# Cameronr11/GAN-Variant-Research

Measured on AMD Instinct MI355X. Metric: images/sec (G+D train step) 256x256 CUT, higher is better.
Workload: dtype bf16; 1 GPU; CUT ResNet-9 G + PatchGAN D + PatchNCE + identity + lazy R1 + DiffAugment, 256x256, batch 16 per GPU (BASELINE.json configs[2]); global_batch=16, parallelism=dp1

## Files before the change

### gan-variant-research_amd/csrc/conv_win7.hip

```cpp
#include "common.h"

namespace {

constexpr int TS = 16, PW = TS + 6, PITCH = 144, PATCH_BYTES = PW * PW * PITCH;
constexpr int NJ = 4;

struct Win7Args {
  const char* in; const char* w; const float* bias; char* out;
  int B, Ho, Wo, tiles_x, tiles_y;
  int in_Hp, in_Wp, in_y0, in_x0, ty0, tx0;
  int out_Hp, out_Wp, out_y0, out_x0;
  int act;
  float* stats;
};

__global__ __launch_bounds__(256, 2) void conv_win7_kernel(Win7Args a) {
  extern __shared__ __attribute__((aligned(16))) char lds[];
  const int tid = threadIdx.x, lane = tid & 63, wave = __builtin_amdgcn_readfirstlane(tid >> 6);
  const int G = gridDim.x;
  const int q = G >> 3, r = G & 7, xcd = blockIdx.x & 7, k = blockIdx.x >> 3;
  const int tile = xcd < r ? xcd * (q + 1) + k : r * (q + 1) + (xcd - r) * q + k;
  const int per_img = a.tiles_x * a.tiles_y;
  const int b = tile / per_img, t2 = tile - b * per_img;
  const int oy0 = (t2 / a.tiles_x) * TS, ox0 = (t2 % a.tiles_x) * TS;

  u32x4_t bw[NJ][7];
  {
    const char* wl = a.w + (lane & 15) * (49 * 128) + (lane >> 4) * 16;
#pragma unroll
    for (int j = 0; j < NJ; ++j) {
      const int id = wave + 4 * j, kx = min(id >> 1, 6), c = id & 1;
#pragma unroll
      for (int ky = 0; ky < 7; ++ky) {
        u32x4_t v = *reinterpret_cast<const u32x4_t*>(wl + (ky * 7 + kx) * 128 + c * 64);
        if (id >= 14) v = u32x4_t{0u, 0u, 0u, 0u};
        bw[j][ky] = v;
      }
    }
  }
  {
    const int ay0 = oy0 + a.in_y0 + a.ty0, ax0 = ox0 + a.in_x0 + a.tx0;
    const char* img = a.in + (int64_t)b * a.in_Hp * a.in_Wp * 128;
    constexpr int NIT = (PW * PW * 8 + 255) / 256;
    u32x4_t st[NIT];
#pragma unroll
    for (int it = 0; it < NIT; ++it) {
      const int i = tid + it * 256;
      const int p = i >> 3, ck = i & 7;
      const int py = p / PW, px = p - py * PW;
      const int ay = ay0 + py, ax = ax0 + px;
      const bool ok = i < PW * PW * 8 && ay >= 0 && ay < a.in_Hp && ax >= 0 && ax < a.in_Wp;
      const int64_t off = ok ? ((int64_t)ay * a.in_Wp + ax) * 128 + ck * 16 : 0;
      u32x4_t v = *reinterpret_cast<const u32x4_t*>(img + off);
      if (!ok) v = u32x4_t{0u, 0u, 0u, 0u};
      st[it] = v;
    }
#pragma unroll
    for (int it = 0; it < NIT; ++it) {
      const int i = tid + it * 256;
      if (i < PW * PW * 8) *reinterpret_cast<u32x4_t*>(lds + (i >> 3) * PITCH + (i & 7) * 16) = st[it];
    }
  }
  __syncthreads();

  f32x4_t acc[TS];
#pragma unroll
  for (int m = 0; m < TS; ++m) acc[m] = f32x4_t{0.f, 0.f, 0.f, 0.f};
  const char* la = lds + (lane & 15) * PITCH + (lane >> 4) * 16;
#pragma unroll
  for (int j = 0; j < NJ; ++j) {
    const int id = wave + 4 * j, kx = min(id >> 1, 6), c = id & 1;
    const char* lj = la + kx * PITCH + c * 64;
#pragma unroll
    for (int R = 0; R < PW; ++R) {
      const u32x4_t xa = *reinterpret_cast<const u32x4_t*>(lj + R * (PW * PITCH));
#pragma unroll
      for (int ky = 0; ky < 7; ++ky) {
        const int m = R - ky;
        if (m >= 0 && m < TS)
          acc[m] = __builtin_amdgcn_mfma_f32_16x16x32_bf16(__builtin_bit_cast(bf16x8_t, bw[j][ky]), __builtin_bit_cast(bf16x8_t, xa), acc[m], 0, 0, 0);
      }
    }
    __builtin_amdgcn_sched_barrier(0);
  }
  __syncthreads();
  {
    float* red = reinterpret_cast<float*>(lds);
#pragma unroll
    for (int m = 0; m < TS; ++m)
      *reinterpret_cast<f32x4_t*>(red + (((wave * TS + m) * TS + (lane & 15)) * 16 + (lane >> 4) * 4)) = acc[m];
  }
  __syncthreads();
  {
    const float* red = reinterpret_cast<const float*>(lds);
    const int m = tid >> 4, x = tid & 15;
    float v[8];
#pragma unroll
    for (int n = 0; n < 8; ++n) v[n] = a.bias ? a.bias[n] : 0.f;
#pragma unroll
    for (int w2 = 0; w2 < 4; ++w2) {
      const f32x4_t p0 = *reinterpret_cast<const f32x4_t*>(red + (((w2 * TS + m) * TS + x) * 16));
      const f32x4_t p1 = *reinterpret_cast<const f32x4_t*>(red + (((w2 * TS + m) * TS + x) * 16 + 4));
      v[0] += p0.x; v[1] += p0.y; v[2] += p0.z; v[3] += p0.w; v[4] += p1.x; v[5] += p1.y; v[6] += p1.z; v[7] += p1.w;
    }
    const int oy = oy0 + m, ox = ox0 + x;
    if (oy < a.Ho && ox < a.Wo) {
#pragma unroll
      for (int n = 0; n < 8; ++n) v[n] = act_apply(v[n], a.act);
      bf16_t* o = reinterpret_cast<bf16_t*>(a.out) + (((int64_t)b * a.out_Hp + oy + a.out_y0) * a.out_Wp + ox + a.out_x0) * 8;
      Chunk<bf16_t>::store(o, v);
    }
  }
}
__device__ __forceinline__ float row16_sum_w7(float v) {
  auto dpp = [](float x, auto ctrl) {
    return __builtin_bit_cast(float, __builtin_amdgcn_update_dpp(0, __builtin_bit_cast(int, x), decltype(ctrl)::value, 0xf, 0xf, true));
  };
  v += dpp(v, std::integral_constant<int, 0xB1>{});
  v += dpp(v, std::integral_constant<int, 0x4E>{});
  v += dpp(v, std::integral_constant<int, 0x141>{});
  v += dpp(v, std::integral_constant<int, 0x140>{});
  return v;
}

constexpr int KS3 = 13;

__global__ __launch_bounds__(256, 2) void conv_win7_from3_kernel(Win7Args a, int wtaps) {
  __shared__ __attribute__((aligned(16))) char lds[(PW * PW + 16) * 16];
  const int tid = threadIdx.x, lane = tid & 63, wave = __builtin_amdgcn_readfirstlane(tid >> 6);
  const int G = gridDim.x;
  const int q = G >> 3, r = G & 7, xcd = blockIdx.x & 7, k = blockIdx.x >> 3;
  const int tile = xcd < r ? xcd * (q + 1) + k : r * (q + 1) + (xcd - r) * q + k;
  const int per_img = a.tiles_x * a.tiles_y;
  const int b = tile / per_img, t2 = tile - b * per_img;
  const int oy0 = (t2 / a.tiles_x) * TS, ox0 = (t2 % a.tiles_x) * TS;
  u32x4_t bw[KS3];
  {
    const char* wl = a.w + ((int64_t)(wave * 16 + (lane & 15)) * wtaps + (lane >> 4)) * 16;
#pragma unroll
    for (int ks = 0; ks < KS3; ++ks) bw[ks] = *reinterpret_cast<const u32x4_t*>(wl + ks * 64);
  }
  {
    const int ay0 = oy0 + a.in_y0 + a.ty0, ax0 = ox0 + a.in_x0 + a.tx0;
    const char* img = a.in + (int64_t)b * a.in_Hp * a.in_Wp * 16;
    u32x4_t st[2];
#pragma unroll
    for (int it = 0; it < 2; ++it) {
      const int p = tid + it * 256;
      const int py = p / PW, px = p - py * PW;
      const int ay = ay0 + py, ax = ax0 + px;
      const bool ok = p < PW * PW && ay >= 0 && ay < a.in_Hp && ax >= 0 && ax < a.in_Wp;
      u32x4_t v = *reinterpret_cast<const u32x4_t*>(img + (ok ? ((int64_t)ay * a.in_Wp + ax) * 16 : 0));
      if (!ok) v = u32x4_t{0u, 0u, 0u, 0u};
      st[it] = v;
    }
#pragma unroll
    for (int it = 0; it < 2; ++it)
      if (tid + it * 256 < PW * PW + 16) *reinterpret_cast<u32x4_t*>(lds + (tid + it * 256) * 16) = st[it];
  }
  __syncthreads();
  f32x4_t acc[TS];
#pragma unroll
  for (int m = 0; m < TS; ++m) acc[m] = f32x4_t{0.f, 0.f, 0.f, 0.f};
  const int g = lane >> 4;
#pragma unroll
  for (int ks = 0; ks < KS3; ++ks) {
    const int t = min(4 * ks + g, 48);
    const int ky = t / 7, kx = t - ky * 7;
    const char* lj = lds + ((ky * PW + kx) + (lane & 15)) * 16;
#pragma unroll
    for (int m = 0; m < TS; ++m) {
      const u32x4_t xa = *reinterpret_cast<const u32x4_t*>(lj + m * (PW * 16));
      acc[m] = __builtin_amdgcn_mfma_f32_16x16x32_bf16(__builtin_bit_cast(bf16x8_t, bw[ks]), __builtin_bit_cast(bf16x8_t, xa), acc[m], 0, 0, 0);
    }
    __builtin_amdgcn_sched_barrier(0);
  }
  const int n0 = wave * 16 + g * 4, x = lane & 15;
  float bias[4];
#pragma unroll
  for (int i = 0; i < 4; ++i) bias[i] = a.bias ? a.bias[n0 + i] : 0.f;
  bf16_t* dst = reinterpret_cast<bf16_t*>(a.out) + (((int64_t)b * a.out_Hp + oy0 + a.out_y0) * a.out_Wp + ox0 + x + a.out_x0) * 64 + n0;
  const bool xok = ox0 + x < a.Wo;
  float ssum[4] = {0.f, 0.f, 0.f, 0.f}, ssq[4] = {0.f, 0.f, 0.f, 0.f};
#pragma unroll
  for (int m = 0; m < TS; ++m) {
    const float v0 = acc[m].x + bias[0], v1 = acc[m].y + bias[1], v2 = acc[m].z + bias[2], v3 = acc[m].w + bias[3];
    uint2 o;
    o.x = (uint32_t)f2bf(v0) | ((uint32_t)f2bf(v1) << 16);
    o.y = (uint32_t)f2bf(v2) | ((uint32_t)f2bf(v3) << 16);
    if (xok && oy0 + m < a.Ho) {
      *reinterpret_cast<uint2*>(dst + (int64_t)m * a.out_Wp * 64) = o;
      ssum[0] += v0; ssum[1] += v1; ssum[2] += v2; ssum[3] += v3;
      ssq[0] += v0 * v0; ssq[1] += v1 * v1; ssq[2] += v2 * v2; ssq[3] += v3 * v3;
    }
  }
  if (a.stats) {
#pragma unroll
    for (int i = 0; i < 4; ++i) { ssum[i] = row16_sum_w7(ssum[i]); ssq[i] = row16_sum_w7(ssq[i]); }
    if (x == 0) {
      float* sp = a.stats + (((int64_t)b * per_img + t2) * 64 + n0) * 2;
#pragma unroll
      for (int i = 0; i < 4; ++i) *reinterpret_cast<float2*>(sp + 2 * i) = make_float2(ssum[i], ssq[i]);
    }
  }
}
}

extern "C" int gan_conv_win7_ok(const gan_conv_desc* d) {
  if (!d || d->dtype != GAN_BF16) return 0;
  const bool to3 = d->Cin == 64 && d->ntaps == 49 && d->Nw == 16 && d->Nst == 8 && d->out_C == 8;
  const bool from3 = d->Cin == 8 && d->ntaps >= 52 && d->Nw == 64 && d->Nst == 64 && d->out_C == 64;
  if (!to3 && !from3) return 0;
  if (d->in_sy != 1 || d->in_sx != 1 || d->out_sy != 1 || d->out_sx != 1 || d->mask || (d->stats && !from3)) return 0;
  if (d->act != GAN_ACT_NONE && !(to3 && d->act == GAN_ACT_TANH)) return 0;
  if (d->max_tapoff != ((d->win_ty0 + 6) * d->in_Wp + d->win_tx0 + 6) * d->Cin) return 0;
  { const char* e = getenv("GAN_NO_WIN7"); if (e && atoi(e)) return 0; }
  return 1;
}

int gan_conv_win7_stats_parts(const gan_conv_desc* d) {
  if (d->w_layout != 2 || d->Cin != 8 || d->Nst != 64 || d->act != GAN_ACT_NONE) return 0;
  return ((d->Wo + TS - 1) / TS) * ((d->Ho + TS - 1) / TS);
}

int gan_conv_win7_launch(const gan_conv_desc* d, hipStream_t s) {
  GAN_CHECK(gan_conv_win7_ok(d), "conv: w_layout 2 set on a descriptor the 7x7 window kernel does not cover");
  GAN_CHECK(d->in_y0 + d->win_ty0 >= 0 && d->in_x0 + d->win_tx0 >= 0 && d->Ho - 1 + d->in_y0 + d->win_ty0 + 6 < d->in_Hp &&
                d->Wo - 1 + d->in_x0 + d->win_tx0 + 6 < d->in_Wp, "conv(7x7 window): taps reach outside the input allocation");
  Win7Args a;
  a.in = (const char*)d->in; a.w = (const char*)d->w; a.bias = d->bias; a.out = (char*)d->out;
  a.B = d->B; a.Ho = d->Ho; a.Wo = d->Wo; a.tiles_x = (d->Wo + TS - 1) / TS; a.tiles_y = (d->Ho + TS - 1) / TS;
  a.in_Hp = d->in_Hp; a.in_Wp = d->in_Wp; a.in_y0 = d->in_y0; a.in_x0 = d->in_x0; a.ty0 = d->win_ty0; a.tx0 = d->win_tx0;
  a.out_Hp = d->out_Hp; a.out_Wp = d->out_Wp; a.out_y0 = d->out_y0; a.out_x0 = d->out_x0;
  a.act = d->act; a.stats = d->stats;
  const int64_t blocks = (int64_t)d->B * a.tiles_x * a.tiles_y;
  GAN_CHECK(blocks < (1ll << 31), "conv(7x7 window): too many tiles");
  static bool attr_set = false;
  if (!attr_set) {
    if (hipFuncSetAttribute((const void*)conv_win7_kernel, hipFuncAttributeMaxDynamicSharedMemorySize, PATCH_BYTES + 64) != hipSuccess)
      return gan_set_error(-2, "conv(7x7 window): cannot raise the dynamic LDS limit to %d bytes", PATCH_BYTES + 64);
    attr_set = true;
  }
  if (d->Cin == 8) {
    hipLaunchKernelGGL(conv_win7_from3_kernel, dim3((unsigned)blocks), dim3(256), 0, s, a, d->ntaps);
    GAN_LAUNCH_CHECK();
    return 0;
  }
  hipLaunchKernelGGL(conv_win7_kernel, dim3((unsigned)blocks), dim3(256), PATCH_BYTES + 64, s, a);
  GAN_LAUNCH_CHECK();
  return 0;
}

namespace {

struct Wg7Args {
  const char* x; const char* g; float* part;
  int B, Ho, Wo, tiles_x, tiles_y, ntiles;
  int x_Hp, x_Wp, x_y0, x_x0;
  int g_Hp, g_Wp, g_y0, g_x0;
};

constexpr int GP = 32;
constexpr int WPITCH = 160, WPATCH = PW * PW * WPITCH;
constexpr int WG7_LDS = WPATCH + 64 + TS * TS * GP;

typedef __attribute__((ext_vector_type(4))) short s16x4_t;

__global__ __launch_bounds__(256, 1) void wgrad_win7_kernel(Wg7Args a) {
  extern __shared__ __attribute__((aligned(16))) char lds[];
  char* lx = lds;
  char* lg = lds + WPATCH + 64;
  const int tid = threadIdx.x, lane = tid & 63, wave = __builtin_amdgcn_readfirstlane(tid >> 6);
  const int fi = lane & 15, fg = lane >> 4, q = fi >> 2, p = fi & 3;
  f32x4_t acc[49];
#pragma unroll
  for (int t = 0; t < 49; ++t) acc[t] = f32x4_t{0.f, 0.f, 0.f, 0.f};
  const int per_img = a.tiles_x * a.tiles_y;
  int xoff[2], goff[2];
#pragma unroll
  for (int h = 0; h < 2; ++h) {
    const int r = fg >> 1, xx = h * 8 + (fg & 1) * 4 + q;
    xoff[h] = (r * PW + xx) * WPITCH + (wave * 16 + p * 4) * 2;
    goff[h] = (r * TS + xx) * GP + p * 8;
  }
  constexpr int NIT = (PW * PW * 8 + 255) / 256;
  u32x4_t st[NIT], gv;
  auto fetch = [&](int tile) {
    const int b = tile / per_img, t2 = tile - b * per_img;
    const int oy0 = (t2 / a.tiles_x) * TS, ox0 = (t2 % a.tiles_x) * TS;
    const int ay0 = oy0 + a.x_y0, ax0 = ox0 + a.x_x0;
    const char* img = a.x + (int64_t)b * a.x_Hp * a.x_Wp * 128;
#pragma unroll
    for (int it = 0; it < NIT; ++it) {
      const int i = tid + it * 256;
      const int px_ = i >> 3, ck = i & 7;
      const int py = px_ / PW, px = px_ - py * PW;
      const int ay = ay0 + py, ax = ax0 + px;
      const bool ok = i < PW * PW * 8 && ay >= 0 && ay < a.x_Hp && ax >= 0 && ax < a.x_Wp;
      u32x4_t v = *reinterpret_cast<const u32x4_t*>(img + (ok ? ((int64_t)ay * a.x_Wp + ax) * 128 + ck * 16 : 0));
      if (!ok) v = u32x4_t{0u, 0u, 0u, 0u};
      st[it] = v;
    }
    const int gy = oy0 + (tid >> 4), gx = ox0 + (tid & 15);
    gv = u32x4_t{0u, 0u, 0u, 0u};
    if (gy < a.Ho && gx < a.Wo) gv = *reinterpret_cast<const u32x4_t*>(a.g + (((int64_t)b * a.g_Hp + gy + a.g_y0) * a.g_Wp + gx + a.g_x0) * 16);
  };
  if ((int)blockIdx.x < a.ntiles) fetch(blockIdx.x);
  for (int tile = blockIdx.x; tile < a.ntiles; tile += gridDim.x) {
    __syncthreads();
#pragma unroll
    for (int it = 0; it < NIT; ++it) {
      const int i = tid + it * 256;
      if (i < PW * PW * 8) *reinterpret_cast<u32x4_t*>(lx + (i >> 3) * WPITCH + (i & 7) * 16) = st[it];
    }
    *reinterpret_cast<u32x4_t*>(lg + tid * GP) = gv;
    *reinterpret_cast<u32x4_t*>(lg + tid * GP + 16) = u32x4_t{0u, 0u, 0u, 0u};
    __syncthreads();
    if (tile + (int)gridDim.x < a.ntiles) fetch(tile + gridDim.x);
    bf16x8_t gfr[8];
#pragma unroll
    for (int ks = 0; ks < 8; ++ks) {
      const s16x4_t g0 = __builtin_amdgcn_ds_read_tr16_b64_v4i16((__attribute__((address_space(3))) s16x4_t*)(lg + ks * (2 * TS * GP) + goff[0]));
      const s16x4_t g1 = __builtin_amdgcn_ds_read_tr16_b64_v4i16((__attribute__((address_space(3))) s16x4_t*)(lg + ks * (2 * TS * GP) + goff[1]));
      gfr[ks] = bf16x8_t{g0[0], g0[1], g0[2], g0[3], g1[0], g1[1], g1[2], g1[3]};
    }
#pragma unroll
    for (int R = 0; R <= 20; ++R) {
#pragma unroll
      for (int kx = 0; kx < 7; ++kx) {
        const int tb = (R * PW + kx) * WPITCH;
        const s16x4_t x0 = __builtin_amdgcn_ds_read_tr16_b64_v4i16((__attribute__((address_space(3))) s16x4_t*)(lx + tb + xoff[0]));
        const s16x4_t x1 = __builtin_amdgcn_ds_read_tr16_b64_v4i16((__attribute__((address_space(3))) s16x4_t*)(lx + tb + xoff[1]));
        const bf16x8_t xv = {x0[0], x0[1], x0[2], x0[3], x1[0], x1[1], x1[2], x1[3]};
#pragma unroll
        for (int ky = R & 1; ky < 7; ky += 2) {
          const int ks = (R - ky) / 2;
          if (R - ky >= 0 && ks < 8) acc[ky * 7 + kx] = __builtin_amdgcn_mfma_f32_16x16x32_bf16(xv, gfr[ks], acc[ky * 7 + kx], 0, 0, 0);
        }
      }
      __builtin_amdgcn_sched_barrier(0);
    }
  }
  if (fi < 8) {
    float* dst = a.part + ((int64_t)blockIdx.x * 8 + fi) * (49 * 64) + wave * 16 + fg * 4;
#pragma unroll
    for (int t = 0; t < 49; ++t) *reinterpret_cast<f32x4_t*>(dst + t * 64) = acc[t];
  }
}
}

namespace {
constexpr int GP64 = 160;
constexpr int XW_BYTES = (PW * PW + 8) * 16;
constexpr int WG7B_LDS = XW_BYTES + TS * TS * GP64;

__global__ __launch_bounds__(256, 2) void wgrad_win7_from3_kernel(Wg7Args a) {
  __shared__ __attribute__((aligned(16))) char lds[WG7B_LDS];
  char* lx = lds;
  char* lg = lds + XW_BYTES;
  const int tid = threadIdx.x, lane = tid & 63, wave = __builtin_amdgcn_readfirstlane(tid >> 6);
  const int fi = lane & 15, fg = lane >> 4, q = fi >> 2, p = fi & 3;
  f32x4_t acc[7][4];
#pragma unroll
  for (int ky = 0; ky < 7; ++ky)
#pragma unroll
    for (int pr = 0; pr < 4; ++pr) acc[ky][pr] = f32x4_t{0.f, 0.f, 0.f, 0.f};
  const int per_img = a.tiles_x * a.tiles_y;
  int xoff[2], goff[2];
#pragma unroll
  for (int h = 0; h < 2; ++h) {
    const int r = fg >> 1, xx = h * 8 + (fg & 1) * 4 + q;
    xoff[h] = (r * PW + xx) * 16 + p * 8;
    goff[h] = (r * TS + xx) * GP64 + (wave * 16 + p * 4) * 2;
  }
  for (int tile = blockIdx.x; tile < a.ntiles; tile += gridDim.x) {
    const int b = tile / per_img, t2 = tile - b * per_img;
    const int oy0 = (t2 / a.tiles_x) * TS, ox0 = (t2 % a.tiles_x) * TS;
    __syncthreads();
    {
      const int ay0 = oy0 + a.x_y0, ax0 = ox0 + a.x_x0;
      const char* img = a.x + (int64_t)b * a.x_Hp * a.x_Wp * 16;
      u32x4_t sx[2];
#pragma unroll
      for (int it = 0; it < 2; ++it) {
        const int px_ = tid + it * 256;
        const int py = px_ / PW, px = px_ - py * PW;
        const int ay = ay0 + py, ax = ax0 + px;
        const bool ok = px_ < PW * PW && ay >= 0 && ay < a.x_Hp && ax >= 0 && ax < a.x_Wp;
        u32x4_t v = *reinterpret_cast<const u32x4_t*>(img + (ok ? ((int64_t)ay * a.x_Wp + ax) * 16 : 0));
        if (!ok) v = u32x4_t{0u, 0u, 0u, 0u};
        sx[it] = v;
      }
      const int gy = oy0 + (tid >> 4), gx = ox0 + (tid & 15);
      const bool gok = gy < a.Ho && gx < a.Wo;
      const char* gp = a.g + (gok ? (((int64_t)b * a.g_Hp + gy + a.g_y0) * a.g_Wp + gx + a.g_x0) * 128 : 0);
      u32x4_t sg[8];
#pragma unroll
      for (int c = 0; c < 8; ++c) { sg[c] = *reinterpret_cast<const u32x4_t*>(gp + c * 16); if (!gok) sg[c] = u32x4_t{0u, 0u, 0u, 0u}; }
#pragma unroll
      for (int it = 0; it < 2; ++it)
        if (tid + it * 256 < PW * PW + 8) *reinterpret_cast<u32x4_t*>(lx + (tid + it * 256) * 16) = sx[it];
#pragma unroll
      for (int c = 0; c < 8; ++c) *reinterpret_cast<u32x4_t*>(lg + tid * GP64 + c * 16) = sg[c];
    }
    __syncthreads();
    bf16x8_t gfr[8];
#pragma unroll
    for (int ks = 0; ks < 8; ++ks) {
      const s16x4_t g0 = __builtin_amdgcn_ds_read_tr16_b64_v4i16((__attribute__((address_space(3))) s16x4_t*)(lg + ks * (2 * TS * GP64) + goff[0]));
      const s16x4_t g1 = __builtin_amdgcn_ds_read_tr16_b64_v4i16((__attribute__((address_space(3))) s16x4_t*)(lg + ks * (2 * TS * GP64) + goff[1]));
      gfr[ks] = bf16x8_t{g0[0], g0[1], g0[2], g0[3], g1[0], g1[1], g1[2], g1[3]};
    }
#pragma unroll
    for (int R = 0; R <= 20; ++R) {
#pragma unroll
      for (int pr = 0; pr < 4; ++pr) {
        const int tb = (R * PW + 2 * pr) * 16;
        const s16x4_t x0 = __builtin_amdgcn_ds_read_tr16_b64_v4i16((__attribute__((address_space(3))) s16x4_t*)(lx + tb + xoff[0]));
        const s16x4_t x1 = __builtin_amdgcn_ds_read_tr16_b64_v4i16((__attribute__((address_space(3))) s16x4_t*)(lx + tb + xoff[1]));
        const bf16x8_t xv = {x0[0], x0[1], x0[2], x0[3], x1[0], x1[1], x1[2], x1[3]};
#pragma unroll
        for (int ky = R & 1; ky < 7; ky += 2) {
          const int ks = (R - ky) / 2;
          if (R - ky >= 0 && ks < 8) acc[ky][pr] = __builtin_amdgcn_mfma_f32_16x16x32_bf16(gfr[ks], xv, acc[ky][pr], 0, 0, 0);
        }
      }
      __builtin_amdgcn_sched_barrier(0);
    }
  }
  const int kxo = fi >> 3, ci = fi & 7;
  float* dst = a.part + ((int64_t)blockIdx.x * 64 + wave * 16 + fg * 4) * (49 * 8) + ci;
#pragma unroll
  for (int ky = 0; ky < 7; ++ky)
#pragma unroll
    for (int pr = 0; pr < 4; ++pr) {
      const int kx = 2 * pr + kxo;
      if (kx < 7) {
        float* o = dst + (ky * 7 + kx) * 8;
        o[0] = acc[ky][pr].x; o[49 * 8] = acc[ky][pr].y; o[2 * 49 * 8] = acc[ky][pr].z; o[3 * 49 * 8] = acc[ky][pr].w;
      }
    }
}
}

extern "C" int gan_wgrad_win7_splits(const gan_wgrad_desc* d) {
  if (!d || d->dtype != GAN_BF16 || d->ntaps != 49) return 0;
  const bool to3 = d->Cx == 64 && d->N == 8 && d->g_C == 8, from3 = d->Cx == 8 && d->N == 64 && d->g_C == 64;
  if (!to3 && !from3) return 0;
  if (d->x_sy != 1 || d->x_sx != 1 || d->g_sy != 1 || d->g_sx != 1) return 0;
  if (d->max_tapoff != (6 * d->x_Wp + 6) * d->Cx) return 0;
  { const char* e = getenv("GAN_NO_WIN7"); if (e && atoi(e)) return 0; }
  const int64_t tiles = (int64_t)d->B * ((d->Ho + TS - 1) / TS) * ((d->Wo + TS - 1) / TS);
  return (int)(tiles < 256 ? tiles : 256);
}

int gan_wgrad_win7_launch(const gan_wgrad_desc* d, hipStream_t s) {
  const int ns = gan_wgrad_win7_splits(d);
  GAN_CHECK(ns > 0 && d->nsplit == ns, "wgrad: variant 2 needs nsplit = gan_wgrad_win7_splits() = %d, got %d", ns, d->nsplit);
  GAN_CHECK(d->x && d->g && d->part, "wgrad(7x7 window): null pointer");
  GAN_CHECK(d->x_y0 >= 0 && d->x_x0 >= 0 && d->Ho - 1 + d->x_y0 + 6 < d->x_Hp && d->Wo - 1 + d->x_x0 + 6 < d->x_Wp,
            "wgrad(7x7 window): taps reach outside the x allocation");
  Wg7Args a;
  a.x = (const char*)d->x; a.g = (const char*)d->g; a.part = d->part;
  a.B = d->B; a.Ho = d->Ho; a.Wo = d->Wo; a.tiles_x = (d->Wo + TS - 1) / TS; a.tiles_y = (d->Ho + TS - 1) / TS;
  a.ntiles = d->B * a.tiles_x * a.tiles_y;
  a.x_Hp = d->x_Hp; a.x_Wp = d->x_Wp; a.x_y0 = d->x_y0; a.x_x0 = d->x_x0;
  a.g_Hp = d->g_Hp; a.g_Wp = d->g_Wp; a.g_y0 = d->g_y0; a.g_x0 = d->g_x0;
  if (d->Cx == 8) {
    hipLaunchKernelGGL(wgrad_win7_from3_kernel, dim3(ns), dim3(256), 0, s, a);
    GAN_LAUNCH_CHECK();
    return 0;
  }
  static bool attr_set = false;
  if (!attr_set) {
    if (hipFuncSetAttribute((const void*)wgrad_win7_kernel, hipFuncAttributeMaxDynamicSharedMemorySize, WG7_LDS) != hipSuccess)
      return gan_set_error(-2, "wgrad(7x7 window): cannot raise the dynamic LDS limit to %d bytes", WG7_LDS);
    attr_set = true;
  }
  hipLaunchKernelGGL(wgrad_win7_kernel, dim3(ns), dim3(256), WG7_LDS, s, a);
  GAN_LAUNCH_CHECK();
  return 0;
}
```

Baseline: 737.9 images/s.

## Restructure 7x7 weight-gradient MFMA to pack ky shifts into K dimension

Replaces the 49 per-tap accumulators in the 7x7 wgrad kernel with a layout where the gradient tile is written to LDS in four row-shifted copies, packing multiple ky offsets into the MFMA K/N lanes. Accumulators shrink to 2x2x7, and the output channels are split into two groups, with the second group skipped when its gradient channels are all zero across the block (checked via __syncthreads_or). This cuts MFMA count and register pressure for the channel-padded case, at the cost of extra LDS writes, a larger LDS footprint and more complex output indexing.

```diff
diff --git a/gan-variant-research_amd/csrc/conv_win7.hip b/gan-variant-research_amd/csrc/conv_win7.hip
--- a/gan-variant-research_amd/csrc/conv_win7.hip
+++ b/gan-variant-research_amd/csrc/conv_win7.hip
@@ -260,21 +260,27 @@
   int g_Hp, g_Wp, g_y0, g_x0;
 };
 
+constexpr int WPITCH = 160, WPATCH = (PW + 1) * PW * WPITCH;
+constexpr int GROWS = TS + 4;
 constexpr int GP = 32;
-constexpr int WPITCH = 160, WPATCH = PW * PW * WPITCH;
-constexpr int WG7_LDS = WPATCH + 64 + TS * TS * GP;
+constexpr int GCOPY = GROWS * TS * GP;
+constexpr int WG7_LDS = WPATCH + 2 * GCOPY;
 
 typedef __attribute__((ext_vector_type(4))) short s16x4_t;
 
 __global__ __launch_bounds__(256, 1) void wgrad_win7_kernel(Wg7Args a) {
   extern __shared__ __attribute__((aligned(16))) char lds[];
   char* lx = lds;
-  char* lg = lds + WPATCH + 64;
+  char* lg = lds + WPATCH;
   const int tid = threadIdx.x, lane = tid & 63, wave = __builtin_amdgcn_readfirstlane(tid >> 6);
   const int fi = lane & 15, fg = lane >> 4, q = fi >> 2, p = fi & 3;
-  f32x4_t acc[49];
-#pragma unroll
-  for (int t = 0; t < 49; ++t) acc[t] = f32x4_t{0.f, 0.f, 0.f, 0.f};
+  f32x4_t acc[2][2][7];
+#pragma unroll
+  for (int cg = 0; cg < 2; ++cg)
+#pragma unroll
+    for (int s = 0; s < 2; ++s)
+#pragma unroll
+      for (int kx = 0; kx < 7; ++kx) acc[cg][s][kx] = f32x4_t{0.f, 0.f, 0.f, 0.f};
   const int per_img = a.tiles_x * a.tiles_y;
   int xoff[2], goff[2];
 #pragma unroll
@@ -283,6 +289,8 @@
     xoff[h] = (r * PW + xx) * WPITCH + (wave * 16 + p * 4) * 2;
     goff[h] = (r * TS + xx) * GP + p * 8;
   }
+  for (int i = tid; i < PW * WPITCH / 16; i += 256) *reinterpret_cast<u32x4_t*>(lx + PW * PW * WPITCH + i * 16) = u32x4_t{0u, 0u, 0u, 0u};
+  for (int i = tid; i < 2 * GCOPY / 16; i += 256) *reinterpret_cast<u32x4_t*>(lg + i * 16) = u32x4_t{0u, 0u, 0u, 0u};
   constexpr int NIT = (PW * PW * 8 + 255) / 256;
   u32x4_t st[NIT], gv;
   auto fetch = [&](int tile) {
@@ -313,39 +321,55 @@
       const int i = tid + it * 256;
       if (i < PW * PW * 8) *reinterpret_cast<u32x4_t*>(lx + (i >> 3) * WPITCH + (i & 7) * 16) = st[it];
     }
-    *reinterpret_cast<u32x4_t*>(lg + tid * GP) = gv;
-    *reinterpret_cast<u32x4_t*>(lg + tid * GP + 16) = u32x4_t{0u, 0u, 0u, 0u};
-    __syncthreads();
+    {
+      const int py = tid >> 4, px = tid & 15;
+#pragma unroll
+      for (int d = 0; d < 4; ++d) {
+        char* gd = lg + ((py + d) * TS + px) * GP + d * 8;
+        *reinterpret_cast<uint2*>(gd) = make_uint2(gv.x, gv.y);
+        *reinterpret_cast<uint2*>(gd + GCOPY) = make_uint2(gv.z, gv.w);
+      }
+    }
+    const int ncg = __syncthreads_or((gv.z | gv.w) != 0u) ? 2 : 1;
     if (tile + (int)gridDim.x < a.ntiles) fetch(tile + gridDim.x);
-    bf16x8_t gfr[8];
-#pragma unroll
-    for (int ks = 0; ks < 8; ++ks) {
-      const s16x4_t g0 = __builtin_amdgcn_ds_read_tr16_b64_v4i16((__attribute__((address_space(3))) s16x4_t*)(lg + ks * (2 * TS * GP) + goff[0]));
-      const s16x4_t g1 = __builtin_amdgcn_ds_read_tr16_b64_v4i16((__attribute__((address_space(3))) s16x4_t*)(lg + ks * (2 * TS * GP) + goff[1]));
-      gfr[ks] = bf16x8_t{g0[0], g0[1], g0[2], g0[3], g1[0], g1[1], g1[2], g1[3]};
-    }
-#pragma unroll
-    for (int R = 0; R <= 20; ++R) {
-#pragma unroll
-      for (int kx = 0; kx < 7; ++kx) {
-        const int tb = (R * PW + kx) * WPITCH;
-        const s16x4_t x0 = __builtin_amdgcn_ds_read_tr16_b64_v4i16((__attribute__((address_space(3))) s16x4_t*)(lx + tb + xoff[0]));
-        const s16x4_t x1 = __builtin_amdgcn_ds_read_tr16_b64_v4i16((__attribute__((address_space(3))) s16x4_t*)(lx + tb + xoff[1]));
-        const bf16x8_t xv = {x0[0], x0[1], x0[2], x0[3], x1[0], x1[1], x1[2], x1[3]};
-#pragma unroll
-        for (int ky = R & 1; ky < 7; ky += 2) {
-          const int ks = (R - ky) / 2;
-          if (R - ky >= 0 && ks < 8) acc[ky * 7 + kx] = __builtin_amdgcn_mfma_f32_16x16x32_bf16(xv, gfr[ks], acc[ky * 7 + kx], 0, 0, 0);
-        }
-      }
-      __builtin_amdgcn_sched_barrier(0);
-    }
-  }
-  if (fi < 8) {
-    float* dst = a.part + ((int64_t)blockIdx.x * 8 + fi) * (49 * 64) + wave * 16 + fg * 4;
-#pragma unroll
-    for (int t = 0; t < 49; ++t) *reinterpret_cast<f32x4_t*>(dst + t * 64) = acc[t];
-  }
+#pragma unroll
+    for (int cg = 0; cg < 2; ++cg) {
+      if (cg >= ncg) break;
+      bf16x8_t gfr[GROWS / 2];
+#pragma unroll
+      for (int ks = 0; ks < GROWS / 2; ++ks) {
+        const char* gk = lg + cg * GCOPY + ks * (2 * TS * GP);
+        const s16x4_t g0 = __builtin_amdgcn_ds_read_tr16_b64_v4i16((__attribute__((address_space(3))) s16x4_t*)(gk + goff[0]));
+        const s16x4_t g1 = __builtin_amdgcn_ds_read_tr16_b64_v4i16((__attribute__((address_space(3))) s16x4_t*)(gk + goff[1]));
+        gfr[ks] = bf16x8_t{g0[0], g0[1], g0[2], g0[3], g1[0], g1[1], g1[2], g1[3]};
+      }
+#pragma unroll
+      for (int ks = 0; ks < GROWS / 2; ++ks) {
+#pragma unroll
+        for (int s = 0; s < 2; ++s)
+#pragma unroll
+          for (int kx = 0; kx < 7; ++kx) {
+            const int tb = ((2 * ks + 3 * s) * PW + kx) * WPITCH;
+            const s16x4_t x0 = __builtin_amdgcn_ds_read_tr16_b64_v4i16((__attribute__((address_space(3))) s16x4_t*)(lx + tb + xoff[0]));
+            const s16x4_t x1 = __builtin_amdgcn_ds_read_tr16_b64_v4i16((__attribute__((address_space(3))) s16x4_t*)(lx + tb + xoff[1]));
+            const bf16x8_t xv = {x0[0], x0[1], x0[2], x0[3], x1[0], x1[1], x1[2], x1[3]};
+            acc[cg][s][kx] = __builtin_amdgcn_mfma_f32_16x16x32_bf16(xv, gfr[ks], acc[cg][s][kx], 0, 0, 0);
+          }
+        __builtin_amdgcn_sched_barrier(0);
+      }
+    }
+  }
+  const int d = fi >> 2;
+  float* dst = a.part + (int64_t)blockIdx.x * (8 * 49 * 64) + wave * 16 + fg * 4;
+#pragma unroll
+  for (int cg = 0; cg < 2; ++cg)
+#pragma unroll
+    for (int s = 0; s < 2; ++s) {
+      if (s == 1 && d == 0) continue;
+      float* o = dst + (4 * cg + (fi & 3)) * (49 * 64) + (3 * s + d) * 7 * 64;
+#pragma unroll
+      for (int kx = 0; kx < 7; ++kx) *reinterpret_cast<f32x4_t*>(o + kx * 64) = acc[cg][s][kx];
+    }
 }
 }
 
```

New measurement: 742.2 images/s (median of 6 runs). No clear change (+0.6%).
